# skyhehe123/SA-SSD

Hardware: AMD Instinct MI355X
Metric: KITTI-Car inference frames/sec (whole job) (higher is better)
Workload: dtype f32; 1 GPU; configs/car_cfg.py inference, fp32, synthetic lidar64 K21 frames (21500 pts -> ~16k voxels), batch=1, random-init SA-SSD weights, points resident in HBM; frames_in_flight=3, spconv_cfg=0, rulebook_pyramid=levels, launch=one hipGraph replay per frame, parallelism=frame-sharded x1, no collective

## Files before the change

include/sassd.h:

```cpp
#ifndef SASSD_H
#define SASSD_H

#include <stddef.h>
#include <stdint.h>

#ifdef __cplusplus
extern "C" {
#endif

#define SASSD_OK       0
#define SASSD_EINVAL  -1
#define SASSD_ENOSPC  -2
#define SASSD_EHIP    -3

#define SASSD_ST_VOXEL_OVERFLOW   1
#define SASSD_ST_HASH_FULL        2
#define SASSD_ST_BOX_OVERFLOW     4
#define SASSD_ST_GRID_SYNC        8

#define SASSD_MAX_POINTS_PER_VOXEL 64

const char *sassd_version(void);
int sassd_last_hip_error(void);
const char *sassd_last_hip_error_string(void);
// ... 96 lines not shown
int sassd_conv2d_wino4_pack_weight(const float *w , int Cout, int Cin, float *packed, void *stream);
size_t sassd_conv2d_wino4_workspace_bytes(int batch, int Cin, int Cout, int H, int W);
int sassd_conv2d_wino4_fwd(const float *x, const float *w_packed, const float *scale, const float *shift, int relu,
                           float *y, int batch, int Cin, int Cout, int H, int W, int cfg, void *workspace,
                           size_t workspace_bytes, void *stream);

int sassd_conv2d_wino4_chain_supported(int Cin, int Cout, int H, int W);
size_t sassd_conv2d_wino4_chain_workspace_bytes(int batch, int cmax, int H, int W);
int sassd_conv2d_wino4_chain(const float *x, int src_products, const float *prev_scale, const float *prev_shift,
                             int prev_relu, const float *w_packed, const float *scale, const float *shift, int relu,
                             float *y, int batch, int Cin, int Cout, int cmax, int H, int W, const int32_t *tile_map,
                             const int32_t *prev_tile_map, int cfg, void *workspace, size_t workspace_bytes,
                             void *stream);
size_t sassd_conv2d_wino4_narrow_packed_floats(int Cin);
int sassd_conv2d_wino4_pack_weight_narrow(const float *w , int Cout, int Cin, float *packed, void *stream);
int sassd_conv2d_wino4_chain_tail(const float *prev_scale, const float *prev_shift, int prev_relu, float *y_prev,
                                  const float *w_packed64, const float *scale, const float *shift, int relu, float *y,
                                  int batch, int Cin, int Cout, int cmax, int H, int W, const int32_t *prev_tile_map, int cfg,
                                  void *workspace, size_t workspace_bytes, void *stream);

size_t sassd_wino4_tile_map_ints(int batch, int H, int W);
int sassd_wino4_tile_map(const int32_t *indices, const int32_t *n_ptr, int cap, int batch, int H, int W,
                         int32_t *tile_map, void *stream);

int sassd_conv1x1_gemm_supported(int Cin, int Cout, int H, int W);
int sassd_conv1x1_gemm_pack_weight(const float *w , int Cout, int Cin, float *packed, void *stream);
int sassd_conv1x1_gemm_fwd(const float *x, const float *w_packed, const float *scale, const float *shift, int relu,
                           float *y, int batch, int Cin, int Cout, int H, int W, int cfg, void *stream);

int sassd_conv2d_bf16_supported(int Cin, int Cout, int H, int W);
size_t sassd_conv2d_bf16_packed_elems(int Cin, int Cout);
int sassd_conv2d_bf16_pack_weight(const float *w, int Cout, int Cin, void *packed, void *stream);
int sassd_conv2d_bf16_fwd(const float *x, const void *w_packed, const float *shift, float *y, int batch, int Cin,
                          int Cout, int H, int W, void *stream);
int sassd_conv2d_bf16_fwd_cfg(const float *x, const void *w_packed, const float *shift, float *y, int batch, int Cin,
                              int Cout, int H, int W, int cfg, void *stream);
int sassd_conv2d_bf16_bnrelu_fwd(const float *x, const float *in_affine, const void *w_packed, const float *shift, float *y,
                                 int batch, int Cin, int Cout, int H, int W, void *stream);

int sassd_conv1x1_bf16_supported(int Cin, int Cout, int HW);
size_t sassd_conv1x1_bf16_packed_elems(int Cin, int Cout);
int sassd_conv1x1_bf16_pack_weight(const float *w, int Cout, int Cin, int transposed, void *packed, void *stream);
int sassd_conv1x1_bf16_fwd(const float *x, const void *w_packed, const float *shift, float *y, int batch, int Cin, int Cout,
                           int HW, void *stream);

int sassd_conv2d_bf16_infer_supported(int Cin, int Cout, int H, int W);
// ... 198 lines not shown
```

sa-ssd_amd/_C.py:

```python
import ctypes as C
import os
import subprocess

_HERE = os.path.dirname(os.path.abspath(__file__))
LIB_PATH = os.path.join(_HERE, "lib", "libsassd.so")
_lib = None

OK, EINVAL, ENOSPC, EHIP = 0, -1, -2, -3
ST_VOXEL_OVERFLOW, ST_HASH_FULL, ST_BOX_OVERFLOW = 1, 2, 4


def build(force=False, verbose=False):
    cmd = ["make", "-C", os.path.join(_HERE, "csrc"), "-j8"]
    if force:
        subprocess.check_call(cmd + ["clean"], stdout=subprocess.DEVNULL)
    out = subprocess.run(cmd, stdout=subprocess.PIPE, stderr=subprocess.STDOUT, text=True)
    if verbose or out.returncode != 0:
        print(out.stdout)
    if out.returncode != 0:
        raise RuntimeError("building libsassd.so failed")
    return LIB_PATH


_SZ = C.c_size_t
# ... 118 lines not shown
    "sassd_bn_relu_fwd": (_I, [_P, _I, _I, _P, _P, _P, _P, _F, _F, _P, _P, _P, _P, _SZ, _P]),
    "sassd_bn_relu_bwd": (_I, [_P, _P, _I, _I, _P, _P, _P, _P, _P, _P, _P, _P, _SZ, _P]),
    "sassd_bn2d_relu_workspace_bytes": (_SZ, [_I]),
    "sassd_bn2d_relu_fwd": (_I, [_P, _I, _I, _I, _P, _P, _P, _P, _F, _F, _P, _P, _P, _P, _SZ, _P]),
    "sassd_bn2d_stats": (_I, [_P, _I, _I, _I, _P, _P, _P, _P, _F, _F, _P, _P, _P, _P, _SZ, _P]),
    "sassd_bn2d_relu_bwd": (_I, [_P, _P, _I, _I, _I, _P, _P, _P, _P, _P, _P, _P, _P, _SZ, _P]),
    "sassd_aux_head_workspace_bytes": (_SZ, [_I]),
    "sassd_aux_prepare": (_I, [_P, _I, _P, _I, _P, _P, _P, _P, _P, _P, _I, _P, _P, _P, _P, _P, _P]),
    "sassd_aux_head_fwd": (_I, [_I, _P, _P, _P, _P, _P, _P, _P, _P, _P, _P, _P, _P, _P, _P, _SZ, _P]),
    "sassd_aux_head_bwd": (_I, [_I, _P, _P, _P, _P, _P, _P, _P, _P, _P, _P, _P, _P, _P, _SZ, _P]),
    "sassd_guided_decode_fwd": (_I, [_P, _P, _P, _I, _P, _P, _P, _P, _I, _I, _I, _I, _P, _P, _P]),
    "sassd_guided_decode_bwd": (_I, [_P, _P, _I, _P, _P, _P, _I, _I, _I, _I, _P, _P, _P]),
    "sassd_boxes_iou3d_batch": (_I, [_P, _P, _I, _I, _P, _P, _I, _P, _P, _P]),
    "sassd_focal_loss_workspace_bytes": (_SZ, [_I]),
    "sassd_focal_loss": (_I, [_P, _P, _I, _P, _I, _P, _P, _P, _SZ, _P]),
    "sassd_conv2d_wino4_chain_supported": (_I, [_I, _I, _I, _I]),
    "sassd_conv2d_wino4_chain_workspace_bytes": (_SZ, [_I, _I, _I, _I]),
    "sassd_conv2d_wino4_chain": (_I, [_P, _I, _P, _P, _I, _P, _P, _P, _I, _P, _I, _I, _I, _I, _I, _I, _P, _P, _I, _P, _SZ, _P]),
    "sassd_conv2d_wino4_narrow_packed_floats": (_SZ, [_I]),
    "sassd_conv2d_wino4_pack_weight_narrow": (_I, [_P, _I, _I, _P, _P]),
    "sassd_conv2d_wino4_chain_tail": (_I, [_P, _P, _I, _P, _P, _P, _P, _I, _P, _I, _I, _I, _I, _I, _I, _P, _I, _P, _SZ, _P]),
    "sassd_wino4_tile_map_ints": (_SZ, [_I, _I, _I]),
    "sassd_wino4_tile_map": (_I, [_P, _P, _I, _I, _I, _I, _P, _P]),
    "sassd_gather_pack": (_I, [_P, _P, _P, C.c_long, _I, _P]),
    "sassd_grad_sumsq": (_I, [_P, C.c_long, _P, _P]),
    "sassd_adam_step": (_I, [_P, _P, _P, _P, C.c_long, _P, _F, _F, _F, _F, _F, _I, _F, _F, _P]),
    "sassd_mfma_probe": (_I, [_P, _P, _P, _P, _P, _P, _I, _P]),
    "sassd_three_interpolate_grad_det_workspace_bytes": (_SZ, [_I, _I]),
    "sassd_three_interpolate_grad_det": (_I, [_I, _I, _I, _P, _P, _P, _P, _P, _SZ, _P]),
    "sassd_aux_head_bwd_det_workspace_bytes": (_SZ, [_I, _P]),
    "sassd_aux_head_bwd_det": (_I, [_I, _P, _P, _P, _P, _P, _P, _P, _P, _P, _P, _P, _P, _P, _SZ, _P]),
    "sassd_pswarp_sample_bwd_det_workspace_bytes": (_SZ, [_I, _I]),
    "sassd_pswarp_sample_bwd_det": (_I, [_P, _I, _I, _I, _P, _P, _I, _F, _F, _F, _P, _P, _P, _P, _SZ, _P]),
    "sassd_grad_sumsq_det_workspace_bytes": (_SZ, [C.c_long]),
    "sassd_grad_sumsq_det": (_I, [_P, C.c_long, _P, _P, _SZ, _P]),
}

EXPORTS = tuple(_SIGS.keys())


def lib():
    global _lib
    if _lib is None:
        if not os.path.exists(LIB_PATH):
            raise RuntimeError("libsassd.so not found at %s -- run `python -c 'import __graft_entry__ as g; "
                               "g.build()'` (there is no CPU fallback)" % LIB_PATH)
# ... 37 lines not shown
```

sa-ssd_amd/csrc/conv2d_wino4.hip:

```cpp
#include "common.h"

namespace {
typedef float f32x16 __attribute__((ext_vector_type(16)));
typedef __bf16 bf16x8 __attribute__((ext_vector_type(8)));
typedef unsigned u32x4 __attribute__((ext_vector_type(4)));
typedef __attribute__((address_space(3))) void *lds_ptr_t;
typedef const __attribute__((address_space(1))) void *glb_ptr_t;

constexpr int kBM = 128, kKC = 32;

__device__ __forceinline__ void g_row(const float g0, const float g1, const float g2, float (&o)[6])
{
    o[0] = g0;
    const float e = g0 + 0.390625f * g2, f = 0.625f * g1;
    o[1] = e + f;
    o[2] = e - f;
    const float e2 = g0 + 2.25f * g2, f2 = 1.5f * g1;
    o[3] = e2 + f2;
    o[4] = e2 - f2;
    o[5] = g2;
}

__global__ void wino4_pack_kernel(const float *__restrict__ w, int Cout, int Cin, float *__restrict__ U, int ldu)
{
// ... 727 lines not shown
    W4Geom G;
    G.B = batch; G.C = Cin; G.H = H; G.W = W; G.TH = H / 4; G.TW = W / 4; G.T = batch * G.TH * G.TW;
    G.Tp = w4_tiles_padded(batch, H, W, 256, geo);
    float *V = (float *)workspace;
    float *M = (float *)((char *)workspace + need / 2);
    int rc;
    if (!(dbg & 128) && (rc = launch_outin(dbg, Cin, batch, w4_plane_bytes(H, W), stream, (const float *)M, G, prev_scale,
                                           prev_shift, prev_relu, w4_plane_pitch(W), V, prev_tile_map, y_prev)))
        return rc;
    W4Gemm P;
    P.U = w_packed64; P.V = V; P.M = M; P.scale = nullptr; P.shift = nullptr; P.relu = 0; P.ncols_dev = nullptr;
    P.np = 36; P.Cin = Cin; P.Cout = 64; P.ldv = G.Tp; P.ldm = G.Tp; P.ncols = G.Tp;
    P.su = (size_t)Cin * 64; P.sv = (size_t)Cin * G.Tp; P.sm = (size_t)64 * G.Tp;
    if (!(dbg & 32) && (rc = launch_w4_gemm<1, 2, 2, kKC, 1>(P, dbg, stream))) return rc;
    W4Geom Go = G;
    Go.C = Cout;
    if (!(dbg & 64))
        hipLaunchKernelGGL(wino4_out_kernel, dim3(cdiv(G.T, 256), Cout), dim3(256), 0, stream, (const float *)M, Go, Cout, 64,
                           scale, shift, relu, y, (const int32_t *)nullptr);
    return sassd_launch_status();
}

namespace {
__global__ void __launch_bounds__(1024) w4_tile_map_kernel(const int32_t *__restrict__ idx, const int32_t *__restrict__ n_ptr,
                                                           int cap, int B, int H, int W, int TH, int TW,
                                                           int32_t *__restrict__ tmap)
{
    extern __shared__ __attribute__((aligned(16))) unsigned char w4_flags[];
    __shared__ int wsum[17];
    const int T = B * TH * TW;
    for (int i = threadIdx.x; i < (T + 3) / 4; i += 1024) ((unsigned *)w4_flags)[i] = 0u;
    __syncthreads();
    const int n = min(*n_ptr, cap);
    for (int r = threadIdx.x; r < n; r += 1024) {
        const int4 c = ((const int4 *)idx)[r];
        if (c.x < 0 || c.x >= B || c.z < 0 || c.z >= H || c.w < 0 || c.w >= W) continue;
        const int ty = c.z >> 2, tx = c.w >> 2;
        const int y0 = ((c.z & 3) == 0 && ty > 0) ? ty - 1 : ty, y1 = ((c.z & 3) == 3 && ty + 1 < TH) ? ty + 1 : ty;
        const int x0 = ((c.w & 3) == 0 && tx > 0) ? tx - 1 : tx, x1 = ((c.w & 3) == 3 && tx + 1 < TW) ? tx + 1 : tx;
        for (int a = y0; a <= y1; ++a)
            for (int e = x0; e <= x1; ++e) w4_flags[(c.x * TH + a) * TW + e] = 1;
    }
    __syncthreads();
    const int per = (T + 1023) / 1024;
    const int t0 = min((int)threadIdx.x * per, T), t1 = min(t0 + per, T);
    int cnt = 0;
    for (int t = t0; t < t1; ++t) cnt += w4_flags[t];
    int total;
    int j = block_exclusive_scan(cnt, wsum, &total);
    for (int t = t0; t < t1; ++t) {
        const bool on = w4_flags[t] != 0;
        tmap[kTmapHead + t] = on ? j : -1;
        if (on) tmap[kTmapHead + T + j++] = t;
    }
    if (threadIdx.x == 0) { tmap[0] = total; tmap[1] = T; tmap[2] = tmap[3] = 0; }
}
}

extern "C" size_t sassd_wino4_tile_map_ints(int batch, int H, int W)
{
    if (batch < 1 || H < 4 || W < 4 || H % 4 || W % 4) return 0;
    const size_t T = (size_t)batch * (H / 4) * (W / 4);
    return T <= 65536 ? kTmapHead + 2 * T : 0;
}

extern "C" int sassd_wino4_tile_map(const int32_t *indices, const int32_t *n_ptr, int cap, int batch, int H, int W,
                                    int32_t *tile_map, void *stream_)
{
    if (!indices || !n_ptr || !tile_map || cap < 1 || sassd_wino4_tile_map_ints(batch, H, W) == 0) return SASSD_EINVAL;
    const int TH = H / 4, TW = W / 4, T = batch * TH * TW;
    hipLaunchKernelGGL(w4_tile_map_kernel, dim3(1), dim3(1024), (size_t)align_up((size_t)T, 16), (hipStream_t)stream_, indices,
                       n_ptr, cap, batch, H, W, TH, TW, tile_map);
    return sassd_launch_status();
}


namespace {
__global__ void conv1x1_pack_kernel(const float *__restrict__ w, int Cout, int Cin, float *__restrict__ U)
{
    const int i = blockIdx.x * blockDim.x + threadIdx.x;
    if (i >= Cout * Cin) return;
    const int co = i % Cout, ci = i / Cout;
    U[(size_t)ci * Cout + co] = w[(size_t)co * Cin + ci];
}
}

extern "C" int sassd_conv1x1_gemm_supported(int Cin, int Cout, int H, int W)
{
    if (!(Cin >= kKC && Cin % kKC == 0 && Cout >= kBM && Cout % kBM == 0 && H > 0 && W > 0)) return 0;
    return w4_pick_wn(H * W, Cout, 1, true) ? 1 : 0;
}

extern "C" int sassd_conv1x1_gemm_pack_weight(const float *w, int Cout, int Cin, float *packed, void *stream_)
{
    if (!w || !packed || Cin < 1 || Cout < 1) return SASSD_EINVAL;
// ... 29 lines not shown
```

sa-ssd_amd/kernels.py:

```python
import numpy as np
import torch

from . import _C

_ws_cache = {}

_weights_gen = [0]


def weights_generation():
    return _weights_gen[0]


def bump_weights_generation():
    _weights_gen[0] += 1


def weight_key(w):
    return (w._version, w.data_ptr(), str(w.device), _weights_gen[0])


_ws_scope = [None]


# ... 489 lines not shown
def wino4_tile_map(indices, n_ptr, cap, batch, h, w, out=None):
    n = _C.lib().sassd_wino4_tile_map_ints(int(batch), int(h), int(w))
    if n == 0:
        return None
    if out is None:
        out = torch.zeros(n, dtype=torch.int32, device=indices.device)
    _C.check(_C.lib().sassd_wino4_tile_map(_C.ptr(indices), _C.ptr(n_ptr), int(cap), int(batch), int(h), int(w), _C.ptr(out),
                                           _C.stream()), "sassd_wino4_tile_map")
    return out


def conv2d_wino4_chain(x, prev, w_packed, cin, cout, cmax, batch, h, w, scale, shift, relu, y, ws, cfg=None, tile_map=None,
                       prev_tile_map=None):
    _chk_cuda(x, w_packed, scale, shift, y, ws)
    ps, pb, pr = prev if prev is not None else (None, None, False)
    _C.check(_C.lib().sassd_conv2d_wino4_chain(_C.ptr(x), 0 if x is not None else 1, _C.ptr(ps), _C.ptr(pb), 1 if pr else 0,
                                               _C.ptr(w_packed), _C.ptr(scale), _C.ptr(shift), 1 if relu else 0,
                                               _C.ptr(y), batch, cin, cout, cmax, h, w, _C.ptr(tile_map), _C.ptr(prev_tile_map),
                                               DEFAULT_CFG["wino4"] if cfg is None else int(cfg), _C.ptr(ws), ws.numel(),
                                               _C.stream()), "sassd_conv2d_wino4_chain")
    return y


def conv2d_wino4_pack_weight_narrow(w):
    _chk_cuda(w)
    cout, cin = w.shape[0], w.shape[1]
    L = _C.lib()
    packed = torch.empty(L.sassd_conv2d_wino4_narrow_packed_floats(cin), dtype=torch.float32, device=w.device)
    _C.check(L.sassd_conv2d_wino4_pack_weight_narrow(_C.ptr(w.contiguous()), cout, cin, _C.ptr(packed), _C.stream()),
             "sassd_conv2d_wino4_pack_weight_narrow")
    return packed


def conv2d_wino4_chain_tail(prev, y_prev, w_packed64, cin, cout, cmax, batch, h, w, scale, shift, relu, y, ws, cfg=None,
                            prev_tile_map=None):
    _chk_cuda(w_packed64, scale, shift, y, ws, y_prev)
    ps, pb, pr = prev
    _C.check(_C.lib().sassd_conv2d_wino4_chain_tail(_C.ptr(ps), _C.ptr(pb), 1 if pr else 0, _C.ptr(y_prev), _C.ptr(w_packed64),
                                                    _C.ptr(scale), _C.ptr(shift), 1 if relu else 0, _C.ptr(y), batch, cin, cout,
                                                    cmax, h, w, _C.ptr(prev_tile_map),
                                                    DEFAULT_CFG["wino4"] if cfg is None else int(cfg), _C.ptr(ws), ws.numel(),
                                                    _C.stream()), "sassd_conv2d_wino4_chain_tail")
    return y


def conv1x1_gemm_supported(cin, cout, h, w):
# ... 707 lines not shown
```

sa-ssd_amd/pipeline.py:

```python
import numpy as np

import torch

from . import kernels as K
from . import anchors as A

BN_EPS = 1e-3

VXNET = [
    ("conv0.0", "conv0.1", "subm", 4, 16, "subm0"), ("conv0.3", "conv0.4", "subm", 16, 16, "subm0"),
    ("down0.0", "down0.1", "down", 16, 32, "down0"),
    ("conv1.0", "conv1.1", "subm", 32, 32, "subm1"), ("conv1.3", "conv1.4", "subm", 32, 32, "subm1"),
    ("down1.0", "down1.1", "down", 32, 64, "down1"),
    ("conv2.0", "conv2.1", "subm", 64, 64, "subm2"), ("conv2.3", "conv2.4", "subm", 64, 64, "subm2"),
    ("conv2.6", "conv2.7", "subm", 64, 64, "subm2"),
    ("down2.0", "down2.1", "down", 64, 64, "down2"),
    ("conv3.0", "conv3.1", "subm", 64, 64, "subm3"), ("conv3.3", "conv3.4", "subm", 64, 64, "subm3"),
    ("conv3.6", "conv3.7", "subm", 64, 64, "subm3"),
    ("extra_conv.0", "extra_conv.1", "1x1", 64, 64, None),
]


def fold_bn(sd, prefix, eps=BN_EPS):
    g, b = sd[prefix + ".weight"].float(), sd[prefix + ".bias"].float()
    m, v = sd[prefix + ".running_mean"].float(), sd[prefix + ".running_var"].float()
    scale = g / torch.sqrt(v + eps)
    return scale.contiguous(), (b - m * scale).contiguous()


def _bev_weight(sd, i, D3):
    w = sd["neck.fcn.conv%d.weight" % i].float()
    if i == 0:
        cout, cin = w.shape[:2]
        c = cin // D3
        w = w.view(cout, c, D3, 3, 3).permute(0, 2, 1, 3, 4).reshape(cout, cin, 3, 3)
    return w.contiguous()


class InferencePlan:

    def __init__(self, state_dict, *, batch_size=1, num_class=1, voxel_size=(0.05, 0.05, 0.1),
                 point_cloud_range=(0, -40., -3., 70.4, 40., 1.), max_num_points=5, max_voxels=20000,
                 sparse_shape=(40, 1600, 1408), anchors=None, anchors_bv=None, anchor_area_threshold=1,
                 anchors_per_loc=2, grid_offsets=(0., 40.), featmap_stride=0.4, rpn_thr=0.1, score_thr=0.3,
                 iou_thr=0.1, cap_k=4096, cap_d=512, device=None, level_cap_factor=2, overlap=True, winograd=True,
                 fused_rulebooks=True, chain_bev=True, pyramid_persistent=False, spconv_cfg=None, wino4_cfg=None,
                 skip_inactive_tiles=True, rb_sync_levels=(0, 1, 2, 3), ps_tail=False, precision="fp32",
                 sparse_precision="fp32"):
        if precision not in ("fp32", "bf16"):
            raise ValueError("precision must be 'fp32' or 'bf16', got %r" % (precision,))
        if sparse_precision not in ("fp32", "bf16"):
            raise ValueError("sparse_precision must be 'fp32' or 'bf16', got %r" % (sparse_precision,))
        self.precision, self.bf16 = precision, precision == "bf16"
        self.sparse_precision, self.sparse_bf16 = sparse_precision, sparse_precision == "bf16"
        dev = torch.device(device if device is not None else "cuda:0")
        self.dev, self.B, self.ncls, self.A = dev, int(batch_size), int(num_class), int(anchors_per_loc)
        self.voxel_size = np.asarray(voxel_size, np.float32)
        self.pc_range = np.asarray(point_cloud_range, np.float32)
        self.T, self.max_voxels = int(max_num_points), int(max_voxels)
        self.shape0 = tuple(int(s) for s in sparse_shape)
        self.rpn_thr, self.score_thr, self.iou_thr = float(rpn_thr), float(score_thr), float(iou_thr)
        self.grid_offsets, self.spatial_scale = grid_offsets, 1.0 / featmap_stride
        self.area_thr = anchor_area_threshold
        self.capK, self.capD = int(cap_k), int(cap_d)
        sd = {k: v.detach().to(dev) for k, v in state_dict.items()}

        self.shapes = [self.shape0]
        for _ in range(3):
            self.shapes.append(K.conv_out_shape(self.shapes[-1]))
        cap0 = self.B * self.max_voxels
        self.caps = [cap0] + [cap0 * level_cap_factor] * 3
# ... 43 lines not shown
            assert an.shape[0] == self.Atot, (an.shape, self.Atot)
            self.anchors = torch.from_numpy(np.ascontiguousarray(an)).to(dev)
            bv = anchors_bv if anchors_bv is not None else A.rbbox2d_to_near_bbox(an[:, [0, 1, 3, 4, 6]])
            self.anchors_bv = torch.from_numpy(np.ascontiguousarray(bv, np.float32)).to(dev)
        else:
            self.anchors = self.anchors_bv = None

        B, H, W = self.B, self.H, self.W
        i32, f32 = torch.int32, torch.float32
        z = lambda *s, dt=f32: torch.zeros(*s, dtype=dt, device=dev)
        self.status = z(1, dt=i32)
        self.row_off = z(B + 1, dt=i32)
        self.vnum = z(B, dt=i32)
        self.n = [self.row_off[B:B + 1]] + [z(1, dt=i32) for _ in range(3)]
        self.idx = [z(c, 4, dt=i32) for c in self.caps]
        self.tables = [K.HashTable(c, dev) for c in self.caps]
        self.nbr = {key: z(self.caps[lvl], 27, dt=i32)
                    for key, lvl in (("subm0", 0), ("down0", 1), ("subm1", 1), ("down1", 2), ("subm2", 2),
                                     ("down2", 3), ("subm3", 3))}
        fdt = torch.bfloat16 if self.sparse_bf16 else f32
        self.feat = [z(max(self.caps), 64, dt=fdt), z(max(self.caps), 64, dt=fdt)]
        self.mean = z(self.caps[0], 4)
        mdt = torch.bfloat16 if self.bf16 else f32
        self.dense = z(B, 64 * D3, H, W, dt=mdt)
        self.act = [z(B, 256, H, W, dt=mdt) for _ in range(3)]
        self.head_out = z(B, self.head_c, H, W)
        self.ps_t = [z(B, self.ps_parts, H, W, dt=mdt), z(B, self.ps_parts, H, W)]
        self.mask = z(B, self.Atot, dt=torch.uint8)
        self.df = dict(guided=z(B, self.capK, 7), labels=z(B, self.capK, dt=i32), scores=z(B, self.capK),
                       counts=z(B, dt=i32))
        self.logits = z(B, self.capK)
        self.det = dict(boxes=z(B, self.capD, 7), scores=z(B, self.capD), labels=z(B, self.capD, dt=i32),
                        counts=z(B, dt=i32))
        self.middle = {}
        self.pyr = None
        if fused_rulebooks:
            self.pyr = K.RulebookPyramid(self.idx, self.n, self.caps, self.shape0, B,
                                         [self.nbr["subm%d" % l] for l in range(4)],
                                         [None] + [self.nbr["down%d" % l] for l in range(3)], self.status)
        self.pyramid_persistent = bool(pyramid_persistent)
        self.spconv_cfg, self.wino4_cfg = spconv_cfg, wino4_cfg
        self.graph = None
        self.record = None
        self._wsid = id(self)
        self.overlap = bool(overlap)
        self.side = torch.cuda.Stream(device=dev) if self.overlap else None
        self.rb_ev = {k: torch.cuda.Event() for k in self.nbr}
        self.mask_ev = torch.cuda.Event()
        self.tile_map = None
        if skip_inactive_tiles and not self.bf16 and self.bev[0][5] == 4:
            n_ints = K._C.lib().sassd_wino4_tile_map_ints(B, H, W)
            if n_ints:
                self.tile_map = z(n_ints, dt=i32)
        self.tmap_ev = torch.cuda.Event()
        self.rb_sync_levels = tuple(sorted(int(l) for l in rb_sync_levels))
        assert self.rb_sync_levels and self.rb_sync_levels[-1] == 3
        self.prof = None
        self.prof_sparse_layers = False

    def _dense_weights_fp32(self, sd, hw, w0, w1, winograd, chain_bev, wino4_cfg, ps_tail):
        D3, dev = self.D3, self.dev
        self.bev = []
        for i in range(8):
            w = _bev_weight(sd, i, D3)
            scale, shift = fold_bn(sd, "neck.fcn.bn%d" % i)
            wino = 0
            if winograd and w.shape[2] == 3:
                if winograd != 2 and K.conv2d_wino4_supported(w.shape[1], w.shape[0], self.H, self.W):
                    wino = 4
                elif K.conv2d_wino_supported(w.shape[1], w.shape[0], self.H, self.W):
                    wino = 2
            if w.shape[2] == 1 and winograd and K.conv1x1_gemm_supported(w.shape[1], w.shape[0], self.H, self.W):
                wino = 1
            wp = (K.conv2d_wino4_pack_weight(w.contiguous()) if wino == 4 else
                  K.conv2d_wino_pack_weight(w.contiguous()) if wino == 2 else
                  K.conv1x1_gemm_pack_weight(w.contiguous()) if wino == 1 else K.conv2d_pack_weight(w.contiguous()))
            self.bev.append((wp, w.shape[0], w.shape[2], scale, shift, wino))
# ... 28 lines not shown
        self.head_narrow = self.ps_narrow = False
        self.bev_cin = [int(sd["neck.fcn.conv%d.weight" % i].shape[1]) for i in range(8)]
        self.bev16 = []
        for i in range(8):
            w = _bev_weight(sd, i, self.D3)
            cout, cin, k = int(w.shape[0]), int(w.shape[1]), int(w.shape[2])
            if k == 3:
                need(K.conv2d_bf16_infer_supported(cin, cout, H, W), "BEV conv%d (3x3, %d -> %d)" % (i, cin, cout))
                wp = K.conv2d_bf16_infer_pack_weight(w)
            else:
                need(k == 1 and K.conv1x1_bf16_infer_supported(cin, cout, H * W),
                     "BEV conv%d (%dx%d, %d -> %d)" % (i, k, k, cin, cout))
                wp = K.conv1x1_bf16_pack_weight(w)
            scale, shift = fold_bn(sd, "neck.fcn.bn%d" % i)
            self.bev16.append((wp, cout, k, scale, shift))
        need(K.conv1x1_bf16_infer_supported(hw.shape[1], hw.shape[0], H * W), "the fused SSD head (%d -> %d)" % (hw.shape[1], hw.shape[0]))
        self.head_w = K.conv1x1_bf16_pack_weight(hw)
        need(w0.shape[2] == 3 and K.conv2d_bf16_infer_supported(w0.shape[1], w0.shape[0], H, W),
             "the part-sensitive conv (%d -> %d)" % (w0.shape[1], w0.shape[0]))
        self.ps_w0 = K.conv2d_bf16_infer_pack_weight(w0)
        need(K.conv1x1_bf16_infer_supported(w1.shape[1], w1.shape[0], H * W), "the part-sensitive 1x1 (%d -> %d)" % (w1.shape[1], w1.shape[0]))
        self.ps_w1 = K.conv1x1_bf16_pack_weight(w1)

    def _ev(self):
        e = torch.cuda.Event(enable_timing=True)
        e.record()
        return e

    def _seg(self, name, e0):
        if self.prof is not None:
            self.prof.setdefault(name, []).append((e0, self._ev()))

    def voxelize(self, clouds, n_dev=None):
        assert len(clouds) == self.B
        e0 = self._ev() if self.prof is not None else None
        self.row_off.fill_(0)
        for b, pts in enumerate(clouds):
            K.voxelize(pts, self.voxel_size, self.pc_range, self.T, self.max_voxels, batch_idx=b, coors_cols=4,
                       want_voxels=False, want_mean=True, nfeat=4,
                       out=dict(coors=self.idx[0], mean=self.mean, voxel_num=self.vnum[b:b + 1],
                                num_points=self._numpts()),
                       row_offset=self.row_off[b:b + 2], status=self.status, cap=self.caps[0],
                       n_dev=None if n_dev is None else n_dev[b:b + 1])
        self._seg("voxelize", e0)

    def _numpts(self):
# ... 22 lines not shown
                self._rulebook_level(lvl)
            return
        self.tables[0].build(self.idx[0], self.n[0], self.shapes[0], B, self.status)
        for lvl in range(4):
            K.rulebook_subm(self.idx[lvl], self.n[lvl], self.caps[lvl], self.shapes[lvl], B, self.tables[lvl],
                            self.nbr["subm%d" % lvl])
            self.rb_ev["subm%d" % lvl].record()
            if lvl < 3:
                K.rulebook_conv(self.idx[lvl], self.n[lvl], self.caps[lvl], self.shapes[lvl], B, self.tables[lvl],
                                self.caps[lvl + 1], self.idx[lvl + 1], self.n[lvl + 1], self.nbr["down%d" % lvl],
                                self.status)
                self.rb_ev["down%d" % lvl].record()
                self.tables[lvl + 1].build(self.idx[lvl + 1], self.n[lvl + 1], self.shapes[lvl + 1], B, self.status)

    def _rulebook_level(self, lvl):
        self.pyr.build(lvl, lvl + 1)
        self.rb_ev["subm%d" % lvl].record()
        if lvl > 0:
            self.rb_ev["down%d" % (lvl - 1)].record()

    def backbone(self, keep_middle=False, anchors_mask=None, densify=True, masks=True, rulebooks=True, convs=True):
        main = torch.cuda.current_stream(self.dev)
        e0 = self._ev() if self.prof is not None else None
        if self.overlap:
            self.side.wait_stream(main)
            with torch.cuda.stream(self.side):
                if rulebooks:
                    self.rulebooks()
                if self.tile_map is not None and densify:
                    K.wino4_tile_map(self.idx[3], self.n[3], self.caps[3], self.B, self.H, self.W, out=self.tile_map)
                    self.tmap_ev.record()
                if masks:
                    self.anchor_masks(anchors_mask)
                self.mask_ev.record()
        else:
            if rulebooks:
                self.rulebooks()
            if self.tile_map is not None and densify:
                K.wino4_tile_map(self.idx[3], self.n[3], self.caps[3], self.B, self.H, self.W, out=self.tile_map)
        if not convs:
            return
        x = self.mean
        lvl = 0
        cur = 0
        covered = -1
        for li, (kind, cin, cout, key, wp, scale, shift) in enumerate(self.sp):
            y = self.feat[cur]
            if kind == "down":
                lvl += 1
            if key is not None and self.overlap and rulebooks and lvl > covered:
                upto = min([l for l in self.rb_sync_levels if l >= lvl] or [3])
                main.wait_event(self.rb_ev["subm%d" % upto])
                covered = upto
            el = self._ev() if self.prof is not None and self.prof_sparse_layers else None
            if self.sparse_bf16:
                K.spconv_fwd_bf16(x, None if key is None else self.nbr[key], self.n[lvl], self.caps[lvl], wp,
                                  1 if key is None else 27, cin, cout, scale, shift, True, y)
            elif kind == "subm" or kind == "down":
                K.spconv_fwd(x, self.nbr[key], self.n[lvl], self.caps[lvl], wp, 27, cin, cout, scale, shift, True, y,
                             cfg=self.spconv_cfg)
            else:
                K.spconv_fwd(x, None, self.n[lvl], self.caps[lvl], wp, 1, cin, cout, scale, shift, True, y, cfg=self.spconv_cfg)
            if el is not None:
                self._seg("sparse_conv%d" % li, el)
            if keep_middle:
                self.middle[li] = (y.clone(), lvl, cout)
            x = y
            cur ^= 1
        self.sp_out = x
        self._seg("sparse", e0)
        if not densify:
            return
        e1 = self._ev() if self.prof is not None else None
        if self.sparse_bf16:
            K.densify_from_bf16(x, self.idx[3], self.n[3], self.caps[3], self.shapes[3], self.B, 1, self.dense, out_bf16=self.bf16)
        elif self.bf16:
            K.densify_bf16(x, self.idx[3], self.n[3], self.caps[3], self.shapes[3], self.B, 1, self.dense)
        else:
            K.densify(x, self.idx[3], self.n[3], self.caps[3], self.shapes[3], self.B, 1, self.dense)
        self._seg("densify", e1)

    def bev_and_heads(self):
        if self.bf16:
            return self._bev_and_heads_bf16()
        x = self.dense
        for i, (wp, cout, ks, scale, shift, wino) in enumerate(self.bev):
            y = self.act[i % 2] if i < 7 else self.act[2]
            e0 = self._ev() if self.prof is not None else None
            if wino == 4:
                keep = (i + 1 < 8 and self.chain[i + 1]) or (i == 6 and self.ps_tail)
                prev = self.bev[i - 1][3:5] + (True,) if self.chain[i] else None
                tmap = self.tile_map if i == 0 else None
                ptmap = self.tile_map if (i == 1 and self.chain[1]) else None
                if tmap is not None and self.overlap:
                    torch.cuda.current_stream(self.dev).wait_event(self.tmap_ev)
                K.conv2d_wino4_chain(None if self.chain[i] else x, prev, wp, self.bev_cin[i], cout, self.cmax, self.B,
                                     self.H, self.W, scale, shift, True, None if keep else y, self.wino4_ws, cfg=self.wino4_cfg,
                                     tile_map=tmap, prev_tile_map=ptmap)
            elif wino == 2:
                K.conv2d_wino_fwd(x, wp, cout, scale, shift, True, y)
            elif wino == 1:
                K.conv1x1_gemm_fwd(x, wp, cout, scale, shift, True, y, cfg=self.wino4_cfg)
            else:
                K.conv2d_fwd(x, wp, cout, ks, scale, shift, True, y)
            if i == 6 and self.ps_tail:
                K.conv2d_wino4_chain_tail(self.bev[6][3:5] + (True,), y, self.ps_w0t, cout, self.ps_parts, self.cmax, self.B,
                                          self.H, self.W, self.ps_s0, self.ps_b0, True, self.ps_t[0], self.wino4_ws,
                                          cfg=self.wino4_cfg)
            self._seg("bev_conv%d" % i, e0)
            x = y
            if i == 6:
                self.conv6 = y
        self.x = x
        e0 = self._ev() if self.prof is not None else None
        if self.head_narrow:
            K.conv1x1_narrow_fwd(x, self.head_w, self.head_c, None, self.head_b, False, self.head_out)
        else:
            K.conv2d_fwd(x, self.head_w, self.head_c, 1, None, self.head_b, False, self.head_out)
        if not self.ps_tail:
            K.conv2d_fwd(self.conv6, self.ps_w0, self.ps_parts, 3, self.ps_s0, self.ps_b0, True, self.ps_t[0])
        if self.ps_narrow:
            K.conv1x1_narrow_fwd(self.ps_t[0], self.ps_w1, self.ps_parts, None, None, False, self.ps_t[1])
        else:
            K.conv2d_fwd(self.ps_t[0], self.ps_w1, self.ps_parts, 1, None, None, False, self.ps_t[1])
        self._seg("heads", e0)

    def _bev_and_heads_bf16(self):
        x = self.dense
        for i, (wp, cout, ks, scale, shift) in enumerate(self.bev16):
            y = self.act[i % 2] if i < 7 else self.act[2]
            e0 = self._ev() if self.prof is not None else None
            if ks == 3:
                K.conv2d_bf16_infer_fwd(x, wp, cout, scale, shift, True, y)
            else:
                K.conv1x1_bf16_infer_fwd(x, wp, cout, scale, shift, True, y)
            self._seg("bev_conv%d" % i, e0)
            x = y
            if i == 6:
                self.conv6 = y
        self.x = x
        e0 = self._ev() if self.prof is not None else None
        K.conv1x1_bf16_infer_fwd(x, self.head_w, self.head_c, None, self.head_b, False, self.head_out, out_bf16=False)
        K.conv2d_bf16_infer_fwd(self.conv6, self.ps_w0, self.ps_parts, self.ps_s0, self.ps_b0, True, self.ps_t[0])
        K.conv1x1_bf16_infer_fwd(self.ps_t[0], self.ps_w1, self.ps_parts, None, None, False, self.ps_t[1], out_bf16=False)
        self._seg("heads", e0)

    def anchor_masks(self, masks=None):
        if masks is not None:
            self.mask.copy_(masks.view(self.B, -1).to(torch.uint8))
            return
        H0, W0 = self.shape0[1], self.shape0[2]
# ... 137 lines not shown
```

Before: 932.8 frames/s.

## Feed first BEV Winograd conv directly from sparse voxels, skip dense scatter

Adds a sparse entry path in which the first BEV Winograd-4 conv gathers input tiles straight from sparse voxel features through a dense index grid. This removes the densify scatter into a large zeroed dense tensor. The tile-map builder is also split from one single-block kernel into a parallel mark kernel plus a multi-block compact/scan kernel, and the same pass now fills the index grid. In exchange, each frame must fill the grid with -1, and gathers read feats indirectly. It is on by default when a tile map exists and BEV conv0 is not chained.

New measurement: 956.0 frames/s, median of 6. 2.5% higher.

```diff
diff --git a/include/sassd.h b/include/sassd.h
--- a/include/sassd.h
+++ b/include/sassd.h
@@ -142,6 +142,14 @@
 size_t sassd_wino4_tile_map_ints(int batch, int H, int W);
 int sassd_wino4_tile_map(const int32_t *indices, const int32_t *n_ptr, int cap, int batch, int H, int W,
                          int32_t *tile_map, void *stream);
+
+size_t sassd_wino4_sparse_grid_ints(int batch, int D, int H, int W);
+int sassd_wino4_sparse_prepare(const int32_t *indices, const int32_t *n_ptr, int cap, int batch, int D, int H, int W,
+                               int32_t *grid, int32_t *tile_map, void *stream);
+int sassd_conv2d_wino4_chain_sparse(const float *feats, int C, int D, const int32_t *grid, const float *w_packed,
+                                    const float *scale, const float *shift, int relu, float *y, int batch, int Cin, int Cout,
+                                    int cmax, int H, int W, const int32_t *tile_map, int cfg, void *workspace,
+                                    size_t workspace_bytes, void *stream);
 
 int sassd_conv1x1_gemm_supported(int Cin, int Cout, int H, int W);
 int sassd_conv1x1_gemm_pack_weight(const float *w , int Cout, int Cin, float *packed, void *stream);
diff --git a/sa-ssd_amd/_C.py b/sa-ssd_amd/_C.py
--- a/sa-ssd_amd/_C.py
+++ b/sa-ssd_amd/_C.py
@@ -164,6 +164,9 @@
     "sassd_conv2d_wino4_chain_tail": (_I, [_P, _P, _I, _P, _P, _P, _P, _I, _P, _I, _I, _I, _I, _I, _I, _P, _I, _P, _SZ, _P]),
     "sassd_wino4_tile_map_ints": (_SZ, [_I, _I, _I]),
     "sassd_wino4_tile_map": (_I, [_P, _P, _I, _I, _I, _I, _P, _P]),
+    "sassd_wino4_sparse_grid_ints": (_SZ, [_I, _I, _I, _I]),
+    "sassd_wino4_sparse_prepare": (_I, [_P, _P, _I, _I, _I, _I, _I, _P, _P, _P]),
+    "sassd_conv2d_wino4_chain_sparse": (_I, [_P, _I, _I, _P, _P, _P, _P, _I, _P, _I, _I, _I, _I, _I, _I, _P, _I, _P, _SZ, _P]),
     "sassd_gather_pack": (_I, [_P, _P, _P, C.c_long, _I, _P]),
     "sassd_grad_sumsq": (_I, [_P, C.c_long, _P, _P]),
     "sassd_adam_step": (_I, [_P, _P, _P, _P, C.c_long, _P, _F, _F, _F, _F, _F, _I, _F, _F, _P]),
diff --git a/sa-ssd_amd/csrc/conv2d_wino4.hip b/sa-ssd_amd/csrc/conv2d_wino4.hip
--- a/sa-ssd_amd/csrc/conv2d_wino4.hip
+++ b/sa-ssd_amd/csrc/conv2d_wino4.hip
@@ -773,38 +773,67 @@
 }
 
 namespace {
-__global__ void __launch_bounds__(1024) w4_tile_map_kernel(const int32_t *__restrict__ idx, const int32_t *__restrict__ n_ptr,
-                                                           int cap, int B, int H, int W, int TH, int TW,
-                                                           int32_t *__restrict__ tmap)
-{
-    extern __shared__ __attribute__((aligned(16))) unsigned char w4_flags[];
+constexpr int kMapBlock = 1024;
+inline size_t w4_flag_off(size_t T) { return align_up(kTmapHead + 2 * T, 4); }
+inline size_t w4_flag_ints(size_t T) { return align_up((T + 3) / 4, 4); }
+
+template <bool SPARSE>
+__global__ void __launch_bounds__(256) w4_mark_kernel(const int32_t *__restrict__ idx, const int32_t *__restrict__ n_ptr, int cap,
+                                                      int B, int D, int H, int W, int TH, int TW,
+                                                      unsigned char *__restrict__ flags, int32_t *__restrict__ grid)
+{
+    const int r = blockIdx.x * 256 + threadIdx.x;
+    if (r >= min(*n_ptr, cap)) return;
+    const int4 c = ((const int4 *)idx)[r];
+    if (c.x < 0 || c.x >= B || c.z < 0 || c.z >= H || c.w < 0 || c.w >= W) return;
+    if (SPARSE) {
+        if (c.y < 0 || c.y >= D) return;
+        grid[(((size_t)c.x * D + c.y) * H + c.z) * W + c.w] = r;
+    }
+    const int ty = c.z >> 2, tx = c.w >> 2;
+    const int y0 = ((c.z & 3) == 0 && ty > 0) ? ty - 1 : ty, y1 = ((c.z & 3) == 3 && ty + 1 < TH) ? ty + 1 : ty;
+    const int x0 = ((c.w & 3) == 0 && tx > 0) ? tx - 1 : tx, x1 = ((c.w & 3) == 3 && tx + 1 < TW) ? tx + 1 : tx;
+    for (int a = y0; a <= y1; ++a)
+        for (int e = x0; e <= x1; ++e) flags[(c.x * TH + a) * TW + e] = 1;
+}
+
+__global__ void __launch_bounds__(kMapBlock) w4_compact_kernel(const unsigned char *__restrict__ flags, int T,
+                                                               int32_t *__restrict__ tmap)
+{
     __shared__ int wsum[17];
-    const int T = B * TH * TW;
-    for (int i = threadIdx.x; i < (T + 3) / 4; i += 1024) ((unsigned *)w4_flags)[i] = 0u;
-    __syncthreads();
-    const int n = min(*n_ptr, cap);
-    for (int r = threadIdx.x; r < n; r += 1024) {
-        const int4 c = ((const int4 *)idx)[r];
-        if (c.x < 0 || c.x >= B || c.z < 0 || c.z >= H || c.w < 0 || c.w >= W) continue;
-        const int ty = c.z >> 2, tx = c.w >> 2;
-        const int y0 = ((c.z & 3) == 0 && ty > 0) ? ty - 1 : ty, y1 = ((c.z & 3) == 3 && ty + 1 < TH) ? ty + 1 : ty;
-        const int x0 = ((c.w & 3) == 0 && tx > 0) ? tx - 1 : tx, x1 = ((c.w & 3) == 3 && tx + 1 < TW) ? tx + 1 : tx;
-        for (int a = y0; a <= y1; ++a)
-            for (int e = x0; e <= x1; ++e) w4_flags[(c.x * TH + a) * TW + e] = 1;
-    }
-    __syncthreads();
-    const int per = (T + 1023) / 1024;
-    const int t0 = min((int)threadIdx.x * per, T), t1 = min(t0 + per, T);
-    int cnt = 0;
-    for (int t = t0; t < t1; ++t) cnt += w4_flags[t];
+    const int t0 = blockIdx.x * kMapBlock;
+    int before = 0;
+    for (int i = threadIdx.x; i < t0 / 16; i += kMapBlock) {
+        const uint4 f = ((const uint4 *)flags)[i];
+        before += __popc(f.x) + __popc(f.y) + __popc(f.z) + __popc(f.w);
+    }
+    int base;
+    block_exclusive_scan(before, wsum, &base);
+    const int t = t0 + threadIdx.x;
+    const int on = t < T ? (int)flags[t] : 0;
     int total;
-    int j = block_exclusive_scan(cnt, wsum, &total);
-    for (int t = t0; t < t1; ++t) {
-        const bool on = w4_flags[t] != 0;
+    const int j = base + block_exclusive_scan(on, wsum, &total);
+    if (t < T) {
         tmap[kTmapHead + t] = on ? j : -1;
-        if (on) tmap[kTmapHead + T + j++] = t;
-    }
-    if (threadIdx.x == 0) { tmap[0] = total; tmap[1] = T; tmap[2] = tmap[3] = 0; }
+        if (on) tmap[kTmapHead + T + j] = t;
+    }
+    if (blockIdx.x == gridDim.x - 1 && threadIdx.x == 0) { tmap[0] = base + total; tmap[1] = T; tmap[2] = tmap[3] = 0; }
+}
+
+template <bool SPARSE>
+int w4_build_map(const int32_t *indices, const int32_t *n_ptr, int cap, int batch, int D, int H, int W, int32_t *grid,
+                 size_t grid_bytes, int32_t *tile_map, hipStream_t stream)
+{
+    const int TH = H / 4, TW = W / 4, T = batch * TH * TW;
+    unsigned char *flags = (unsigned char *)(tile_map + w4_flag_off(T));
+    int rc = SPARSE ? sassd_fill2(grid, grid_bytes, 0xFF, flags, w4_flag_ints(T) * 4, 0, stream)
+                    : sassd_fill2(flags, w4_flag_ints(T) * 4, 0, flags, 0, 0, stream);
+    if (rc) return rc;
+    hipLaunchKernelGGL(w4_mark_kernel<SPARSE>, dim3(cdiv(cap, 256)), dim3(256), 0, stream, indices, n_ptr, cap, batch, D, H, W,
+                       TH, TW, flags, grid);
+    hipLaunchKernelGGL(w4_compact_kernel, dim3(cdiv(T, kMapBlock)), dim3(kMapBlock), 0, stream, (const unsigned char *)flags, T,
+                       tile_map);
+    return sassd_launch_status();
 }
 }
 
@@ -812,16 +841,154 @@
 {
     if (batch < 1 || H < 4 || W < 4 || H % 4 || W % 4) return 0;
     const size_t T = (size_t)batch * (H / 4) * (W / 4);
-    return T <= 65536 ? kTmapHead + 2 * T : 0;
+    return T <= ((size_t)1 << 24) ? w4_flag_off(T) + w4_flag_ints(T) : 0;
 }
 
 extern "C" int sassd_wino4_tile_map(const int32_t *indices, const int32_t *n_ptr, int cap, int batch, int H, int W,
                                     int32_t *tile_map, void *stream_)
 {
     if (!indices || !n_ptr || !tile_map || cap < 1 || sassd_wino4_tile_map_ints(batch, H, W) == 0) return SASSD_EINVAL;
-    const int TH = H / 4, TW = W / 4, T = batch * TH * TW;
-    hipLaunchKernelGGL(w4_tile_map_kernel, dim3(1), dim3(1024), (size_t)align_up((size_t)T, 16), (hipStream_t)stream_, indices,
-                       n_ptr, cap, batch, H, W, TH, TW, tile_map);
+    if (((uintptr_t)tile_map & 15) || ((uintptr_t)indices & 15)) return SASSD_EINVAL;
+    return w4_build_map<false>(indices, n_ptr, cap, batch, 1, H, W, nullptr, 0, tile_map, (hipStream_t)stream_);
+}
+
+namespace {
+__global__ void __launch_bounds__(256) wino4_in_sparse_kernel(const float *__restrict__ feats, int C, int D,
+                                                              const int32_t *__restrict__ grid, W4Geom G,
+                                                              float *__restrict__ V, const int32_t *__restrict__ tmap)
+{
+    __shared__ __attribute__((aligned(16))) float tr[2][36 * 256];
+    const int t0 = blockIdx.x * 256;
+    const int nt = tmap[0];
+    if (t0 >= nt) return;
+    const int j = t0 + threadIdx.x;
+    const int cq = C >> 2;
+    const int d = blockIdx.y / cq, c0 = (blockIdx.y - d * cq) * 4;
+    int row[6][6];
+    bool any = false;
+    if (j < nt) {
+        const int t = tmap[kTmapHead + G.T + j];
+        const int tpi = G.TH * G.TW;
+        const int b = t / tpi, r = t - b * tpi;
+        const int ty = r / G.TW, tx = r - ty * G.TW;
+        const int32_t *src = grid + ((size_t)b * D + d) * G.H * G.W;
+        const int y0 = 4 * ty - 1, x0 = 4 * tx - 1;
+#pragma unroll
+        for (int i = 0; i < 6; ++i) {
+            const int yy = y0 + i;
+            const bool rok = yy >= 0 && yy < G.H;
+#pragma unroll
+            for (int k = 0; k < 6; ++k) {
+                const int xx = x0 + k;
+                row[i][k] = (rok && xx >= 0 && xx < G.W) ? src[(size_t)yy * G.W + xx] : -1;
+                any |= row[i][k] >= 0;
+            }
+        }
+    }
+    float4 d4[6][6];
+    if (any) {
+#pragma unroll
+        for (int i = 0; i < 6; ++i)
+#pragma unroll
+            for (int k = 0; k < 6; ++k)
+                d4[i][k] = row[i][k] >= 0 ? *reinterpret_cast<const float4 *>(feats + (size_t)row[i][k] * C + c0)
+                                          : make_float4(0.f, 0.f, 0.f, 0.f);
+    }
+    const size_t plane = (size_t)G.C * G.Tp;
+    const int c4 = threadIdx.x & 63;
+    const bool st = t0 + c4 * 4 < G.Tp;
+#pragma unroll
+    for (int ch = 0; ch < 4; ++ch) {
+        float *buf = tr[ch & 1];
+        if (any) {
+            float u[6][6];
+#pragma unroll
+            for (int k = 0; k < 6; ++k) {
+                float col[6];
+#pragma unroll
+                for (int i = 0; i < 6; ++i)
+                    col[i] = ch == 0 ? d4[i][k].x : ch == 1 ? d4[i][k].y : ch == 2 ? d4[i][k].z : d4[i][k].w;
+                float o[6];
+                bt_vec(col, o);
+#pragma unroll
+                for (int i = 0; i < 6; ++i) u[i][k] = o[i];
+            }
+#pragma unroll
+            for (int i = 0; i < 6; ++i) {
+                float o[6];
+                bt_vec(u[i], o);
+#pragma unroll
+                for (int k = 0; k < 6; ++k) buf[(i * 6 + k) * 256 + threadIdx.x] = o[k];
+            }
+        } else {
+#pragma unroll
+            for (int p = 0; p < 36; ++p) buf[p * 256 + threadIdx.x] = 0.f;
+        }
+        __syncthreads();
+        if (st) {
+            float *dst = V + ((size_t)d * C + c0 + ch) * G.Tp + t0 + c4 * 4;
+#pragma unroll
+            for (int k = 0; k < 9; ++k) {
+                const int p = (threadIdx.x >> 6) + 4 * k;
+                *reinterpret_cast<float4 *>(dst + (size_t)p * plane) = *reinterpret_cast<const float4 *>(buf + p * 256 + c4 * 4);
+            }
+        }
+    }
+}
+}
+
+extern "C" size_t sassd_wino4_sparse_grid_ints(int batch, int D, int H, int W)
+{
+    if (batch < 1 || D < 1 || D > 8 || H < 4 || W < 4 || H % 4 || W % 4) return 0;
+    return (size_t)batch * D * H * W;
+}
+
+extern "C" int sassd_wino4_sparse_prepare(const int32_t *indices, const int32_t *n_ptr, int cap, int batch, int D, int H, int W,
+                                          int32_t *grid, int32_t *tile_map, void *stream_)
+{
+    if (!indices || !n_ptr || !grid || !tile_map || cap < 1 || sassd_wino4_tile_map_ints(batch, H, W) == 0) return SASSD_EINVAL;
+    const size_t gi = sassd_wino4_sparse_grid_ints(batch, D, H, W);
+    if (gi == 0) return SASSD_EINVAL;
+    if (((uintptr_t)tile_map & 15) || ((uintptr_t)indices & 15) || ((uintptr_t)grid & 15)) return SASSD_EINVAL;
+    return w4_build_map<true>(indices, n_ptr, cap, batch, D, H, W, grid, gi * 4, tile_map, (hipStream_t)stream_);
+}
+
+extern "C" int sassd_conv2d_wino4_chain_sparse(const float *feats, int C, int D, const int32_t *grid, const float *w_packed,
+                                               const float *scale, const float *shift, int relu, float *y, int batch, int Cin,
+                                               int Cout, int cmax, int H, int W, const int32_t *tile_map, int cfg,
+                                               void *workspace, size_t workspace_bytes, void *stream_)
+{
+    const int geo = w4_geo(cfg), dbg = w4_dbg(cfg);
+    if (!feats || !grid || !tile_map || !w_packed || !workspace || batch < 1 || C < 4 || C % 4 || D < 1 || D > 8) return SASSD_EINVAL;
+    if ((long long)C * D != Cin || Cin % kKC || !sassd_conv2d_wino4_supported(Cin, Cout, H, W) || cmax < Cin || cmax < Cout)
+        return SASSD_EINVAL;
+    if (((uintptr_t)feats & 15) || ((uintptr_t)grid & 15) || ((uintptr_t)tile_map & 15) || (y && ((uintptr_t)y & 15)) ||
+        ((uintptr_t)w_packed & 15) || ((uintptr_t)workspace & 15))
+        return SASSD_EINVAL;
+    const size_t need = sassd_conv2d_wino4_chain_workspace_bytes(batch, cmax, H, W);
+    if (need == 0 || workspace_bytes < need) return SASSD_ENOSPC;
+    hipStream_t stream = (hipStream_t)stream_;
+    W4Geom G;
+    G.B = batch; G.C = Cin; G.H = H; G.W = W; G.TH = H / 4; G.TW = W / 4; G.T = batch * G.TH * G.TW;
+    G.Tp = w4_tiles_padded(batch, H, W, Cout, geo);
+    float *V = (float *)workspace;
+    float *M = (float *)((char *)workspace + need / 2);
+    if (!(dbg & 16))
+        hipLaunchKernelGGL(wino4_in_sparse_kernel, dim3(cdiv(G.T, 256), D * (C / 4)), dim3(256), 0, stream, feats, C, D, grid, G, V,
+                           tile_map);
+    W4Gemm P;
+    P.U = w_packed; P.V = V; P.M = M; P.scale = nullptr; P.shift = nullptr; P.relu = 0; P.ncols_dev = tile_map;
+    P.np = 36; P.Cin = Cin; P.Cout = Cout; P.ldv = G.Tp; P.ldm = G.Tp; P.ncols = G.Tp;
+    P.su = (size_t)Cin * Cout; P.sv = (size_t)Cin * G.Tp; P.sm = (size_t)Cout * G.Tp;
+    int rc = SASSD_OK;
+    if (!(dbg & 32)) rc = w4_launch(w4_tile(G.T, Cout, geo), P, dbg, stream);
+    if (rc) return rc;
+    if (y && !(dbg & 64)) {
+        W4Geom Go = G;
+        Go.C = Cout;
+        hipLaunchKernelGGL(wino4_out_kernel, dim3(cdiv(G.T, 256), Cout), dim3(256), 0, stream, (const float *)M, Go, Cout, Cout,
+                           scale, shift, relu, y, tile_map);
+    }
     return sassd_launch_status();
 }
 
diff --git a/sa-ssd_amd/kernels.py b/sa-ssd_amd/kernels.py
--- a/sa-ssd_amd/kernels.py
+++ b/sa-ssd_amd/kernels.py
@@ -535,6 +535,29 @@
     return y
 
 
+def wino4_sparse_grid(batch, d, h, w, device):
+    n = _C.lib().sassd_wino4_sparse_grid_ints(int(batch), int(d), int(h), int(w))
+    return torch.full((n,), -1, dtype=torch.int32, device=device) if n else None
+
+
+def wino4_sparse_prepare(indices, n_ptr, cap, batch, d, h, w, grid, tile_map):
+    _chk_cuda(indices, n_ptr, grid, tile_map)
+    _C.check(_C.lib().sassd_wino4_sparse_prepare(_C.ptr(indices), _C.ptr(n_ptr), int(cap), int(batch), int(d), int(h), int(w),
+                                                 _C.ptr(grid), _C.ptr(tile_map), _C.stream()), "sassd_wino4_sparse_prepare")
+    return grid, tile_map
+
+
+def conv2d_wino4_chain_sparse(feats, d, grid, w_packed, cin, cout, cmax, batch, h, w, scale, shift, relu, y, ws, tile_map,
+                              cfg=None):
+    _chk_cuda(feats, grid, w_packed, scale, shift, y, ws, tile_map)
+    _C.check(_C.lib().sassd_conv2d_wino4_chain_sparse(_C.ptr(feats), int(feats.shape[1]), int(d), _C.ptr(grid), _C.ptr(w_packed),
+                                                      _C.ptr(scale), _C.ptr(shift), 1 if relu else 0, _C.ptr(y), batch, cin,
+                                                      cout, cmax, h, w, _C.ptr(tile_map),
+                                                      DEFAULT_CFG["wino4"] if cfg is None else int(cfg), _C.ptr(ws), ws.numel(),
+                                                      _C.stream()), "sassd_conv2d_wino4_chain_sparse")
+    return y
+
+
 def conv2d_wino4_pack_weight_narrow(w):
     _chk_cuda(w)
     cout, cin = w.shape[0], w.shape[1]
diff --git a/sa-ssd_amd/pipeline.py b/sa-ssd_amd/pipeline.py
--- a/sa-ssd_amd/pipeline.py
+++ b/sa-ssd_amd/pipeline.py
@@ -46,7 +46,7 @@
                  iou_thr=0.1, cap_k=4096, cap_d=512, device=None, level_cap_factor=2, overlap=True, winograd=True,
                  fused_rulebooks=True, chain_bev=True, pyramid_persistent=False, spconv_cfg=None, wino4_cfg=None,
                  skip_inactive_tiles=True, rb_sync_levels=(0, 1, 2, 3), ps_tail=False, precision="fp32",
-                 sparse_precision="fp32"):
+                 sparse_precision="fp32", dense_entry=False):
         if precision not in ("fp32", "bf16"):
             raise ValueError("precision must be 'fp32' or 'bf16', got %r" % (precision,))
         if sparse_precision not in ("fp32", "bf16"):
@@ -136,7 +136,8 @@
         self.feat = [z(max(self.caps), 64, dt=fdt), z(max(self.caps), 64, dt=fdt)]
         self.mean = z(self.caps[0], 4)
         mdt = torch.bfloat16 if self.bf16 else f32
-        self.dense = z(B, 64 * D3, H, W, dt=mdt)
+        self._dense_shape, self._dense_dt = (B, 64 * D3, H, W), mdt
+        self._dense = None
         self.act = [z(B, 256, H, W, dt=mdt) for _ in range(3)]
         self.head_out = z(B, self.head_c, H, W)
         self.ps_t = [z(B, self.ps_parts, H, W, dt=mdt), z(B, self.ps_parts, H, W)]
@@ -167,6 +168,14 @@
             if n_ints:
                 self.tile_map = z(n_ints, dt=i32)
         self.tmap_ev = torch.cuda.Event()
+        self.sparse_grid = None
+        if not dense_entry and self.tile_map is not None and not self.sparse_bf16 and not self.chain[0]:
+            self.sparse_grid = K.wino4_sparse_grid(B, D3, H, W, dev)
+        self.sparse_entry = self.sparse_grid is not None
+        self._sparse_frame = False
+        self._tmap_joined = False
+        if not self.sparse_entry:
+            self._dense_map()
         self.rb_sync_levels = tuple(sorted(int(l) for l in rb_sync_levels))
         assert self.rb_sync_levels and self.rb_sync_levels[-1] == 3
         self.prof = None
@@ -241,6 +250,17 @@
         need(K.conv1x1_bf16_infer_supported(w1.shape[1], w1.shape[0], H * W), "the part-sensitive 1x1 (%d -> %d)" % (w1.shape[1], w1.shape[0]))
         self.ps_w1 = K.conv1x1_bf16_pack_weight(w1)
 
+    def _dense_map(self):
+        if self._dense is None:
+            self._dense = torch.zeros(*self._dense_shape, dtype=self._dense_dt, device=self.dev)
+        return self._dense
+
+    @property
+    def dense(self):
+        if self._sparse_frame:
+            K.densify(self.sp_out, self.idx[3], self.n[3], self.caps[3], self.shapes[3], self.B, 1, self._dense_map())
+        return self._dense_map()
+
     def _ev(self):
         e = torch.cuda.Event(enable_timing=True)
         e.record()
@@ -309,13 +329,15 @@
     def backbone(self, keep_middle=False, anchors_mask=None, densify=True, masks=True, rulebooks=True, convs=True):
         main = torch.cuda.current_stream(self.dev)
         e0 = self._ev() if self.prof is not None else None
+        sparse = self.sparse_entry and densify and not keep_middle
+        self._sparse_frame, self._tmap_joined = sparse, False
         if self.overlap:
             self.side.wait_stream(main)
             with torch.cuda.stream(self.side):
                 if rulebooks:
                     self.rulebooks()
                 if self.tile_map is not None and densify:
-                    K.wino4_tile_map(self.idx[3], self.n[3], self.caps[3], self.B, self.H, self.W, out=self.tile_map)
+                    self._tile_map(sparse)
                     self.tmap_ev.record()
                 if masks:
                     self.anchor_masks(anchors_mask)
@@ -323,8 +345,8 @@
         else:
             if rulebooks:
                 self.rulebooks()
-            if self.tile_map is not None and densify:
-                K.wino4_tile_map(self.idx[3], self.n[3], self.caps[3], self.B, self.H, self.W, out=self.tile_map)
+            if self.tile_map is not None and densify and not sparse:
+                self._tile_map(False)
         if not convs:
             return
         x = self.mean
@@ -359,18 +381,32 @@
         if not densify:
             return
         e1 = self._ev() if self.prof is not None else None
-        if self.sparse_bf16:
-            K.densify_from_bf16(x, self.idx[3], self.n[3], self.caps[3], self.shapes[3], self.B, 1, self.dense, out_bf16=self.bf16)
+        if sparse:
+            if self.overlap:
+                main.wait_event(self.tmap_ev)
+                self._tmap_joined = True
+            else:
+                self._tile_map(True)
+        elif self.sparse_bf16:
+            K.densify_from_bf16(x, self.idx[3], self.n[3], self.caps[3], self.shapes[3], self.B, 1, self._dense_map(),
+                                  out_bf16=self.bf16)
         elif self.bf16:
-            K.densify_bf16(x, self.idx[3], self.n[3], self.caps[3], self.shapes[3], self.B, 1, self.dense)
-        else:
-            K.densify(x, self.idx[3], self.n[3], self.caps[3], self.shapes[3], self.B, 1, self.dense)
+            K.densify_bf16(x, self.idx[3], self.n[3], self.caps[3], self.shapes[3], self.B, 1, self._dense_map())
+        else:
+            K.densify(x, self.idx[3], self.n[3], self.caps[3], self.shapes[3], self.B, 1, self._dense_map())
         self._seg("densify", e1)
+
+    def _tile_map(self, sparse):
+        if sparse:
+            K.wino4_sparse_prepare(self.idx[3], self.n[3], self.caps[3], self.B, self.D3, self.H, self.W, self.sparse_grid,
+                                   self.tile_map)
+        else:
+            K.wino4_tile_map(self.idx[3], self.n[3], self.caps[3], self.B, self.H, self.W, out=self.tile_map)
 
     def bev_and_heads(self):
         if self.bf16:
             return self._bev_and_heads_bf16()
-        x = self.dense
+        x = None if self._sparse_frame else self._dense_map()
         for i, (wp, cout, ks, scale, shift, wino) in enumerate(self.bev):
             y = self.act[i % 2] if i < 7 else self.act[2]
             e0 = self._ev() if self.prof is not None else None
@@ -379,11 +415,16 @@
                 prev = self.bev[i - 1][3:5] + (True,) if self.chain[i] else None
                 tmap = self.tile_map if i == 0 else None
                 ptmap = self.tile_map if (i == 1 and self.chain[1]) else None
-                if tmap is not None and self.overlap:
+                if tmap is not None and self.overlap and not self._tmap_joined:
                     torch.cuda.current_stream(self.dev).wait_event(self.tmap_ev)
-                K.conv2d_wino4_chain(None if self.chain[i] else x, prev, wp, self.bev_cin[i], cout, self.cmax, self.B,
-                                     self.H, self.W, scale, shift, True, None if keep else y, self.wino4_ws, cfg=self.wino4_cfg,
-                                     tile_map=tmap, prev_tile_map=ptmap)
+                if i == 0 and self._sparse_frame:
+                    K.conv2d_wino4_chain_sparse(self.sp_out, self.D3, self.sparse_grid, wp, self.bev_cin[0], cout, self.cmax,
+                                                self.B, self.H, self.W, scale, shift, True, None if keep else y, self.wino4_ws,
+                                                tmap, cfg=self.wino4_cfg)
+                else:
+                    K.conv2d_wino4_chain(None if self.chain[i] else x, prev, wp, self.bev_cin[i], cout, self.cmax, self.B,
+                                         self.H, self.W, scale, shift, True, None if keep else y, self.wino4_ws,
+                                         cfg=self.wino4_cfg, tile_map=tmap, prev_tile_map=ptmap)
             elif wino == 2:
                 K.conv2d_wino_fwd(x, wp, cout, scale, shift, True, y)
             elif wino == 1:
@@ -413,7 +454,7 @@
         self._seg("heads", e0)
 
     def _bev_and_heads_bf16(self):
-        x = self.dense
+        x = self._dense_map()
         for i, (wp, cout, ks, scale, shift) in enumerate(self.bev16):
             y = self.act[i % 2] if i < 7 else self.act[2]
             e0 = self._ev() if self.prof is not None else None
```
